# truongp-aws/neuronx-distributed-llama3_2

Hardware: AMD Instinct MI355X
Metric: tokens/sec (whole node) Llama-3-8B TP=8 bf16 training at 1/2/4/8 MI355X (higher is better)
Workload: dtype bf16

## Files before the change

### neuronx_distributed_llama3_2_amd/csrc/dense_gemm.hip

```cpp
#include "common.h"

#include <cstdlib>
#include <type_traits>

namespace nxd {
namespace dg {

constexpr int BM = 256, BN = 256, BK = 64, NT = 512;
constexpr int REG = 16384;
constexpr int BUF = 4 * REG;
constexpr int LDS_BYTES = 2 * BUF;
constexpr int R_ALO = 0, R_AHI = REG, R_BLO = 2 * REG, R_BHI = 3 * REG;

enum Layout { LNT = 0, LTN = 1 };
enum Epi { BF16 = 0, F32_ACC = 1, F32_ATOMIC = 2 };

struct Params {
  const uint16_t* a;
  const uint16_t* b;
  void* c;
  int M, N, K;
  int64_t lda, ldb, ldc;
  int mt, nt;
  int splits;
  int k_per_split;
  int band;
};

typedef __attribute__((address_space(3))) char lds_char_t;
typedef __attribute__((address_space(3))) short4_t lds_short4_t;
__device__ __forceinline__ uint32_t lds_addr(const char* q) { return (uint32_t)(uintptr_t)(const lds_char_t*)q; }

__device__ __forceinline__ void dma16(const void* src, uint32_t lds_dst) {
  uint32_t sv;
  asm volatile("s_mov_b32 %0, m0\n\ts_mov_b32 m0, %2\n\ts_nop 0\n\tglobal_load_lds_dwordx4 %1, off\n\ts_mov_b32 m0, %0"
               : "=&s"(sv) : "v"(src), "s"(lds_dst) : "memory");
}

__device__ __forceinline__ int nt_swz(int r) { return (r >> 1) & 7; }
__device__ __forceinline__ int tn_swz(int t) { return 2 * ((t & 3) | (((t >> 3) & 1) << 2)); }

__device__ __forceinline__ bf16x8_t frag_nt(const char* reg, int r0, int s) {
  const int l = threadIdx.x & 63, r = r0 + (l & 15), ch = (l >> 4) + 4 * s;
  return __builtin_bit_cast(bf16x8_t, *reinterpret_cast<const u32x4_t*>(reg + r * 128 + ((ch ^ nt_swz(r)) << 4)));
}
__device__ __forceinline__ bf16x8_t frag_tn(const char* reg, int f0, int s) {
  const int l = threadIdx.x & 63, g = l >> 4, i = l & 15, q = i >> 2, p = i & 3;
  const int col = f0 + 4 * p, t = 32 * s + 8 * g + q;
  const char* b0 = reg + t * 256 + (((col >> 3) ^ tn_swz(t)) << 4) + 8 * (p & 1);
  const char* b1 = reg + (t + 4) * 256 + (((col >> 3) ^ tn_swz(t + 4)) << 4) + 8 * (p & 1);
  const short4_t lo = __builtin_amdgcn_ds_read_tr16_b64_v4i16((lds_short4_t*)b0);
  const short4_t hi = __builtin_amdgcn_ds_read_tr16_b64_v4i16((lds_short4_t*)b1);
  const short __attribute__((ext_vector_type(8))) a8 = {lo[0], lo[1], lo[2], lo[3], hi[0], hi[1], hi[2], hi[3]};
  return __builtin_bit_cast(bf16x8_t, a8);
}

template <int L>
__device__ __forceinline__ bf16x8_t frag(const char* reg, int x0, int s) {
  if constexpr (L == LNT) return frag_nt(reg, x0, s);
  else return frag_tn(reg, x0, s);
}

__device__ __forceinline__ void barrier() {
  __builtin_amdgcn_sched_barrier(0);
  __builtin_amdgcn_s_barrier();
  __builtin_amdgcn_sched_barrier(0);
}

__device__ __forceinline__ void wait_regions(int younger) {
  switch (younger) {
    case 5: asm volatile("s_waitcnt vmcnt(10)" ::: "memory"); break;
    case 4: asm volatile("s_waitcnt vmcnt(8)" ::: "memory"); break;
    case 3: asm volatile("s_waitcnt vmcnt(6)" ::: "memory"); break;
    case 2: asm volatile("s_waitcnt vmcnt(4)" ::: "memory"); break;
    case 1: asm volatile("s_waitcnt vmcnt(2)" ::: "memory"); break;
    default: asm volatile("s_waitcnt vmcnt(0)" ::: "memory"); break;
  }
}

template <int L, int E, int PIPE>
__global__ void __launch_bounds__(NT, 1) gemm_kernel(Params p) {
  __shared__ __attribute__((aligned(16))) char smem[LDS_BYTES];
  const int tiles = p.mt * p.nt;
  const int id = xcd_remap(blockIdx.x, gridDim.x);
  const int split = id / tiles;
  int rt, ct;
  {
    const int within = id - split * tiles;
    const int kb = p.band, bnd = within / (kb * p.nt), rem = within - bnd * kb * p.nt;
    const int h = min(kb, p.mt - bnd * kb);
    rt = bnd * kb + rem % h;
    ct = rem / h;
  }
  const int m0 = rt * BM, n0 = ct * BN;
  const int k_begin = split * p.k_per_split;
  const int k_end = min(p.K, k_begin + p.k_per_split);
  const int nk = (k_end - k_begin) / BK;

  const int wid = threadIdx.x >> 6, lane = threadIdx.x & 63;
  const int wr = wid >> 2, wc = wid & 3;

  f32x4_t acc[4][4][2];
#pragma unroll
  for (int q = 0; q < 4; ++q)
#pragma unroll
    for (int i = 0; i < 4; ++i)
#pragma unroll
      for (int j = 0; j < 2; ++j) acc[q][i][j] = f32x4_t{0.f, 0.f, 0.f, 0.f};

  const uint16_t* sa[2][2];
// ... 14 lines not shown
      }
    }
  const int64_t adv_a = L == LNT ? (int64_t)BK : (int64_t)BK * p.lda;
  const int64_t adv_b = L == LNT ? (int64_t)BK : (int64_t)BK * p.ldb;
  const uint32_t lds0 = lds_addr(smem);

  auto issue = [&](auto rc, int s) {
    constexpr int R = decltype(rc)::value;
    if (s >= nk) return;
    const uint32_t dst = lds0 + (s & 1) * BUF + (R == 0 ? R_ALO : R == 1 ? R_BLO : R == 2 ? R_BHI : R_AHI) + wid * 2048;
    if constexpr (R == 0 || R == 3) {
      constexpr int h = R == 0 ? 0 : 1;
      const int64_t o = (int64_t)s * adv_a;
      dma16(sa[h][0] + o, __builtin_amdgcn_readfirstlane(dst));
      dma16(sa[h][1] + o, __builtin_amdgcn_readfirstlane(dst + 1024));
    } else {
      constexpr int h = R == 1 ? 0 : 1;
      const int64_t o = (int64_t)s * adv_b;
      dma16(sb[h][0] + o, __builtin_amdgcn_readfirstlane(dst));
      dma16(sb[h][1] + o, __builtin_amdgcn_readfirstlane(dst + 1024));
    }
  };
  const int last = 4 * nk - 1;
  auto wait_for = [&](int need, int max_younger = 4) {
    if (need > last) return;
    wait_regions(min(max_younger, last - need));
  };

  using I0 = std::integral_constant<int, 0>;
  using I1 = std::integral_constant<int, 1>;
  using I2 = std::integral_constant<int, 2>;
  using I3 = std::integral_constant<int, 3>;
  bf16x8_t af[4][2], blo[2][2], bhi[2][2];
  auto mfma_q = [&](auto qc, bf16x8_t (&bf)[2][2]) {
    constexpr int qd = decltype(qc)::value;
    __builtin_amdgcn_s_setprio(1);
#pragma unroll
    for (int s = 0; s < 2; ++s)
#pragma unroll
      for (int i = 0; i < 4; ++i)
#pragma unroll
        for (int j = 0; j < 2; ++j)
          acc[qd][i][j] = __builtin_amdgcn_mfma_f32_16x16x32_bf16(af[i][s], bf[j][s], acc[qd][i][j], 0, 0, 0);
    __builtin_amdgcn_s_setprio(0);
  };

  if constexpr (PIPE == 0) {
  issue(I0{}, 0); issue(I1{}, 0); issue(I2{}, 0); issue(I3{}, 0); issue(I0{}, 1); issue(I1{}, 1);
  wait_for(1);
  barrier();
  const bool grp1 = wr == 1;
  if (grp1) barrier();
  for (int t = 0; t < nk; ++t) {
    const char* buf = smem + (t & 1) * BUF;
    issue(I2{}, t + 1);
#pragma unroll
    for (int i = 0; i < 4; ++i)
#pragma unroll
      for (int s = 0; s < 2; ++s) af[i][s] = frag<L>(buf + R_ALO, wr * 64 + 16 * i, s);
#pragma unroll
    for (int j = 0; j < 2; ++j)
#pragma unroll
      for (int s = 0; s < 2; ++s) blo[j][s] = frag<L>(buf + R_BLO, wc * 32 + 16 * j, s);
    if (grp1) wait_for(4 * t + 2);
    barrier();
    mfma_q(I0{}, blo);
    if (!grp1) wait_for(4 * t + 2);
    barrier();
    issue(I3{}, t + 1);
#pragma unroll
    for (int j = 0; j < 2; ++j)
#pragma unroll
      for (int s = 0; s < 2; ++s) bhi[j][s] = frag<L>(buf + R_BHI, wc * 32 + 16 * j, s);
    if (grp1) wait_for(4 * t + 3);
    barrier();
    mfma_q(I1{}, bhi);
    if (!grp1) wait_for(4 * t + 3);
    barrier();
    issue(I0{}, t + 2);
#pragma unroll
    for (int i = 0; i < 4; ++i)
#pragma unroll
      for (int s = 0; s < 2; ++s) af[i][s] = frag<L>(buf + R_AHI, wr * 64 + 16 * i, s);
    barrier();
    mfma_q(I2{}, bhi);
    barrier();
    issue(I1{}, t + 2);
    if (grp1) wait_for(4 * t + 5);
    barrier();
    mfma_q(I3{}, blo);
    if (!grp1) wait_for(4 * t + 5);
    barrier();
  }
  if (!grp1) barrier();
  } else {
    issue(I0{}, 0); issue(I1{}, 0); issue(I2{}, 0); issue(I3{}, 0); issue(I0{}, 1); issue(I1{}, 1); issue(I2{}, 1);
    wait_for(1, 5);
    barrier();
#pragma unroll
    for (int i = 0; i < 4; ++i)
#pragma unroll
      for (int s = 0; s < 2; ++s) af[i][s] = frag<L>(smem + R_ALO, wr * 64 + 16 * i, s);
#pragma unroll
    for (int j = 0; j < 2; ++j)
#pragma unroll
      for (int s = 0; s < 2; ++s) blo[j][s] = frag<L>(smem + R_BLO, wc * 32 + 16 * j, s);
    wait_for(2);
    barrier();
    for (int t = 0; t < nk; ++t) {
      const char* buf = smem + (t & 1) * BUF;
      const char* nbuf = smem + ((t + 1) & 1) * BUF;
      issue(I3{}, t + 1);
#pragma unroll
      for (int s = 0; s < 2; ++s)
#pragma unroll
        for (int i = 0; i < 4; ++i) {
#pragma unroll
          for (int j = 0; j < 2; ++j)
            acc[0][i][j] = __builtin_amdgcn_mfma_f32_16x16x32_bf16(af[i][s], blo[j][s], acc[0][i][j], 0, 0, 0);
          if (i < 2) bhi[i][s] = frag<L>(buf + R_BHI, wc * 32 + 16 * i, s);
        }
      wait_for(4 * t + 3);
      barrier();
      issue(I0{}, t + 2);
#pragma unroll
      for (int s = 0; s < 2; ++s)
#pragma unroll
        for (int i = 0; i < 4; ++i) {
#pragma unroll
          for (int j = 0; j < 2; ++j)
            acc[1][i][j] = __builtin_amdgcn_mfma_f32_16x16x32_bf16(af[i][s], bhi[j][s], acc[1][i][j], 0, 0, 0);
          af[i][s] = frag<L>(buf + R_AHI, wr * 64 + 16 * i, s);
        }
      barrier();
      issue(I1{}, t + 2);
#pragma unroll
      for (int s = 0; s < 2; ++s)
#pragma unroll
        for (int i = 0; i < 4; ++i)
#pragma unroll
          for (int j = 0; j < 2; ++j)
            acc[2][i][j] = __builtin_amdgcn_mfma_f32_16x16x32_bf16(af[i][s], bhi[j][s], acc[2][i][j], 0, 0, 0);
      wait_for(4 * t + 5);
      barrier();
      issue(I2{}, t + 2);
#pragma unroll
      for (int s = 0; s < 2; ++s)
#pragma unroll
        for (int j = 0; j < 2; ++j) {
#pragma unroll
          for (int i = 0; i < 4; ++i) {
            acc[3][i][j] = __builtin_amdgcn_mfma_f32_16x16x32_bf16(af[i][s], blo[j][s], acc[3][i][j], 0, 0, 0);
            if (j == 1) af[i][s] = frag<L>(nbuf + R_ALO, wr * 64 + 16 * i, s);
          }
          blo[j][s] = frag<L>(nbuf + R_BLO, wc * 32 + 16 * j, s);
        }
      wait_for(4 * t + 6);
      barrier();
    }
  }
  asm volatile("s_waitcnt vmcnt(0)" ::: "memory");
  __syncthreads();

  constexpr int LD = 36;
  float* slab = reinterpret_cast<float*>(smem) + wid * (64 * LD);
  const int crow = 4 * (lane >> 4), ccol = lane & 15;
#pragma unroll
  for (int qd = 0; qd < 4; ++qd) {
    const int rh = (qd == 2 || qd == 3) ? 1 : 0, ch = (qd == 1 || qd == 2) ? 1 : 0;
#pragma unroll
    for (int i = 0; i < 4; ++i)
#pragma unroll
      for (int j = 0; j < 2; ++j)
#pragma unroll
        for (int r = 0; r < 4; ++r) slab[(16 * i + crow + r) * LD + 16 * j + ccol] = acc[qd][i][j][r];
    __builtin_amdgcn_wave_barrier();
    const int row0 = m0 + 128 * rh + 64 * wr, col0 = n0 + 128 * ch + 32 * wc;
    if constexpr (E == F32_ATOMIC) {
      const int col = col0 + (lane & 31);
      float* cp = static_cast<float*>(p.c);
#pragma unroll 8
      for (int rr = 0; rr < 32; ++rr) {
        const int lr = 2 * rr + (lane >> 5), row = row0 + lr;
        const float v = slab[lr * LD + (lane & 31)];
        if (row < p.M && col < p.N) unsafeAtomicAdd(cp + (int64_t)row * p.ldc + col, v);
      }
    } else {
#pragma unroll
      for (int ps = 0; ps < 4; ++ps) {
        const int lr = 16 * ps + (lane >> 2), c8 = 8 * (lane & 3);
        const int row = row0 + lr, col = col0 + c8;
        const f32x4_t v0 = *reinterpret_cast<const f32x4_t*>(slab + lr * LD + c8);
        const f32x4_t v1 = *reinterpret_cast<const f32x4_t*>(slab + lr * LD + c8 + 4);
        if (row < p.M && col < p.N) {
          if constexpr (E == BF16) {
            u32x4_t o;
            o[0] = pack2bf(v0[0], v0[1]); o[1] = pack2bf(v0[2], v0[3]);
            o[2] = pack2bf(v1[0], v1[1]); o[3] = pack2bf(v1[2], v1[3]);
            *reinterpret_cast<u32x4_t*>(static_cast<uint16_t*>(p.c) + (int64_t)row * p.ldc + col) = o;
          } else {
            f32x4_t* cp = reinterpret_cast<f32x4_t*>(static_cast<float*>(p.c) + (int64_t)row * p.ldc + col);
            const f32x4_t c0 = cp[0], c1 = cp[1];
            cp[0] = c0 + v0;
            cp[1] = c1 + v1;
          }
        }
      }
    }
    __builtin_amdgcn_wave_barrier();
  }
}

constexpr int NT4 = 256;

__device__ __forceinline__ int tn4_swz(int t) { return ((t & 3) << 2) | ((t >> 2) & 3); }

template <int L>
__device__ __forceinline__ bf16x8_t frag32(const char* reg, int x0, int ks) {
  const int l = threadIdx.x & 63;
  if constexpr (L == LNT) {
    const int r = x0 + (l & 31), ch = 2 * ks + (l >> 5);
    return __builtin_bit_cast(bf16x8_t, *reinterpret_cast<const u32x4_t*>(reg + r * 128 + ((ch ^ nt_swz(r)) << 4)));
  } else {
    const int g = l >> 4, q = (l >> 2) & 3, pp = l & 3;
    const int t = 16 * ks + 8 * (g >> 1) + q;
    const int ch = (x0 >> 3) + 2 * (g & 1) + (pp >> 1);
    const char* b0 = reg + t * 256 + ((ch ^ tn4_swz(t)) << 4) + 8 * (pp & 1);
    const char* b1 = reg + (t + 4) * 256 + ((ch ^ tn4_swz(t + 4)) << 4) + 8 * (pp & 1);
    const short4_t lo = __builtin_amdgcn_ds_read_tr16_b64_v4i16((lds_short4_t*)b0);
    const short4_t hi = __builtin_amdgcn_ds_read_tr16_b64_v4i16((lds_short4_t*)b1);
    const short __attribute__((ext_vector_type(8))) a8 = {lo[0], lo[1], lo[2], lo[3], hi[0], hi[1], hi[2], hi[3]};
    return __builtin_bit_cast(bf16x8_t, a8);
  }
}

template <int L, int E>
__global__ void __launch_bounds__(NT4, 1) gemm4_kernel(Params p) {
  __shared__ __attribute__((aligned(16))) char smem[LDS_BYTES];
  const int tiles = p.mt * p.nt;
  const int id = xcd_remap(blockIdx.x, gridDim.x);
  const int split = id / tiles;
  int rt, ct;
  {
    const int within = id - split * tiles;
    const int kb = p.band, bnd = within / (kb * p.nt), rem = within - bnd * kb * p.nt;
    const int h = min(kb, p.mt - bnd * kb);
    rt = bnd * kb + rem % h;
    ct = rem / h;
  }
  const int m0 = rt * BM, n0 = ct * BN;
  const int k_begin = split * p.k_per_split;
  const int k_end = min(p.K, k_begin + p.k_per_split);
  const int nk = (k_end - k_begin) / BK;
  const int wid = threadIdx.x >> 6, lane = threadIdx.x & 63;
  const int wr = wid >> 1, wc = wid & 1;

  f32x16_t acc[4][4];
#pragma unroll
  for (int i = 0; i < 4; ++i)
#pragma unroll
    for (int j = 0; j < 4; ++j)
#pragma unroll
      for (int r = 0; r < 16; ++r) acc[i][j][r] = 0.f;

  constexpr int NV = L == LNT ? 2 : 4;
  const uint16_t* sa[NV];
  const uint16_t* sb[NV];
#pragma unroll
  for (int v = 0; v < NV; ++v) {
    if constexpr (L == LNT) {
      const int pr = 8 * (4 * wid + v) + (lane >> 3), c = (lane & 7) ^ nt_swz(pr);
      sa[v] = p.a + (int64_t)(m0 + pr) * p.lda + k_begin + 8 * c;
      sb[v] = p.b + (int64_t)(n0 + pr) * p.ldb + k_begin + 8 * c;
    } else {
      const int pr = 4 * (4 * wid + v) + (lane >> 4), c = (lane & 15) ^ tn4_swz(pr);
      sa[v] = p.a + (int64_t)(k_begin + pr) * p.lda + m0 + 8 * c;
      sb[v] = p.b + (int64_t)(k_begin + pr) * p.ldb + n0 + 8 * c;
    }
  }
  auto pv = [](int j) { return L == LNT ? (j & 1) : j; };
  auto poff = [&](int h, int j, int64_t ld) -> int64_t {
    if constexpr (L == LNT) return (int64_t)(128 * h + 8 * (j & ~1)) * ld;
    else return (int64_t)128 * h;
  };
  const int64_t adv_a = L == LNT ? (int64_t)BK : (int64_t)BK * p.lda;
  const int64_t adv_b = L == LNT ? (int64_t)BK : (int64_t)BK * p.ldb;
  const uint32_t lds0 = lds_addr(smem);
  auto issue_piece = [&](int s, int q) {
    const int r = q >> 2, j = q & 3, h = r & 1;
    const uint32_t dst = lds0 + (s & 1) * BUF + (r == 0 ? R_ALO : r == 1 ? R_AHI : r == 2 ? R_BLO : R_BHI) + wid * 4096 + j * 1024;
    const uint16_t* src = r < 2 ? sa[pv(j)] + (int64_t)s * adv_a + poff(h, j, p.lda)
                                : sb[pv(j)] + (int64_t)s * adv_b + poff(h, j, p.ldb);
    dma16(src, __builtin_amdgcn_readfirstlane(dst));
  };
  const int ra = wr ? R_AHI : R_ALO, rb = wc ? R_BHI : R_BLO;
  bf16x8_t fa0[4], fb0[4], fa1[4], fb1[4];
  auto rd = [&](const char* buf, int ks, bf16x8_t (&fa)[4], bf16x8_t (&fb)[4]) {
#pragma unroll
    for (int i = 0; i < 4; ++i) fa[i] = frag32<L>(buf + ra, 32 * i, ks);
#pragma unroll
    for (int j = 0; j < 4; ++j) fb[j] = frag32<L>(buf + rb, 32 * j, ks);
  };
  auto mm = [&](bf16x8_t (&fa)[4], bf16x8_t (&fb)[4]) {
#pragma unroll
    for (int i = 0; i < 4; ++i)
#pragma unroll
      for (int j = 0; j < 4; ++j) acc[i][j] = __builtin_amdgcn_mfma_f32_32x32x16_bf16(fa[i], fb[j], acc[i][j], 0, 0, 0);
  };

#pragma unroll
  for (int q = 0; q < 16; ++q) issue_piece(0, q);
  if (nk > 1) {
#pragma unroll
    for (int q = 0; q < 16; ++q) issue_piece(1, q);
    asm volatile("s_waitcnt vmcnt(16)" ::: "memory");
  } else {
    asm volatile("s_waitcnt vmcnt(0)" ::: "memory");
  }
  barrier();
  rd(smem, 0, fa0, fb0);
  for (int t = 0; t < nk; ++t) {
    const char* buf = smem + (t & 1) * BUF;
    rd(buf, 1, fa1, fb1);
    mm(fa0, fb0);
    rd(buf, 2, fa0, fb0);
    mm(fa1, fb1);
    rd(buf, 3, fa1, fb1);
    mm(fa0, fb0);
    asm volatile("s_waitcnt lgkmcnt(0)" ::: "memory");
    asm volatile("s_waitcnt vmcnt(0)" ::: "memory");
    barrier();
    rd(smem + ((t + 1) & 1) * BUF, 0, fa0, fb0);
    if (t + 2 < nk) {
#pragma unroll
      for (int q = 0; q < 16; ++q) issue_piece(t + 2, q);
    }
    mm(fa1, fb1);
  }
  asm volatile("s_waitcnt vmcnt(0)" ::: "memory");
  __syncthreads();

  constexpr int LD = 132;
  float* slab = reinterpret_cast<float*>(smem) + wid * (32 * LD);
#pragma unroll
  for (int i = 0; i < 4; ++i) {
#pragma unroll
    for (int j = 0; j < 4; ++j)
#pragma unroll
      for (int r = 0; r < 16; ++r)
        slab[((r & 3) + 8 * (r >> 2) + 4 * (lane >> 5)) * LD + 32 * j + (lane & 31)] = acc[i][j][r];
    __builtin_amdgcn_wave_barrier();
    const int row0 = m0 + 128 * wr + 32 * i, col0 = n0 + 128 * wc;
    if constexpr (E == F32_ATOMIC) {
      float* cp = static_cast<float*>(p.c);
#pragma unroll 2
      for (int rr = 0; rr < 64; ++rr) {
        const int lr = rr >> 1, col = col0 + 64 * (rr & 1) + lane, row = row0 + lr;
        const float v = slab[lr * LD + 64 * (rr & 1) + lane];
        if (row < p.M && col < p.N) unsafeAtomicAdd(cp + (int64_t)row * p.ldc + col, v);
      }
    } else {
#pragma unroll
      for (int ps = 0; ps < 8; ++ps) {
        const int lr = 4 * ps + (lane >> 4), c8 = 8 * (lane & 15);
        const int row = row0 + lr, col = col0 + c8;
        const f32x4_t v0 = *reinterpret_cast<const f32x4_t*>(slab + lr * LD + c8);
        const f32x4_t v1 = *reinterpret_cast<const f32x4_t*>(slab + lr * LD + c8 + 4);
        if (row < p.M && col < p.N) {
          if constexpr (E == BF16) {
            u32x4_t o;
            o[0] = pack2bf(v0[0], v0[1]); o[1] = pack2bf(v0[2], v0[3]);
            o[2] = pack2bf(v1[0], v1[1]); o[3] = pack2bf(v1[2], v1[3]);
            *reinterpret_cast<u32x4_t*>(static_cast<uint16_t*>(p.c) + (int64_t)row * p.ldc + col) = o;
          } else {
            f32x4_t* cp = reinterpret_cast<f32x4_t*>(static_cast<float*>(p.c) + (int64_t)row * p.ldc + col);
            const f32x4_t c0 = cp[0], c1 = cp[1];
            cp[0] = c0 + v0;
            cp[1] = c1 + v1;
          }
        }
      }
    }
    __builtin_amdgcn_wave_barrier();
  }
}

static int g_pipe = -1;

static int env_int(const char* name, int dflt) {
  const char* e = getenv(name);
  return e ? atoi(e) : dflt;
}

}

void dense_gemm_set_pipe(int v) { dg::g_pipe = v; }

// ... 8 lines not shown
    const int64_t cost = (int64_t)ceil_div(tiles * s, 256) * (ceil_div(steps, s) + 6);
    if (cost * 10 < best_cost * 9 && cost < best_cost) {
      best_cost = cost;
      best = s;
    }
  }
  return best;
}

int dense_gemm_launch(int layout, int epi, const void* a, int64_t lda, const void* b, int64_t ldb, void* c, int64_t ldc,
                      int M, int N, int K, int splits, hipStream_t stream) {
  if (M <= 0 || N <= 0 || K <= 0) return 0;
  if (K % dg::BK || N % 8 || lda % 8 || ldb % 8 || ldc % 4) return -1;
  if (layout == dg::LTN && M % 8) return -1;
  if (epi == dg::BF16 && ldc % 8) return -1;
  dg::Params p{};
  p.a = static_cast<const uint16_t*>(a);
  p.b = static_cast<const uint16_t*>(b);
  p.c = c;
  p.M = M; p.N = N; p.K = K;
  p.lda = lda; p.ldb = ldb; p.ldc = ldc;
  p.mt = ceil_div(M, dg::BM);
  p.nt = ceil_div(N, dg::BN);
  const int steps = K / dg::BK;
  if (epi != dg::F32_ATOMIC) splits = 1;
  else if (splits <= 0) splits = dense_gemm_choose_splits(M, N, K);
  splits = splits < 1 ? 1 : (splits > steps ? steps : splits);
  p.k_per_split = ceil_div(steps, splits) * dg::BK;
  p.splits = ceil_div(K, p.k_per_split);
  static const int band = [] { const int v = dg::env_int("NXD_DG_BAND", 8); return v > 0 ? v : 8; }();
  p.band = band;
  const int64_t nwg = (int64_t)p.mt * p.nt * p.splits;
  if (nwg > INT32_MAX) return -2;
  static int pipe_env = dg::env_int("NXD_DG_PIPE", 1);
  int pipe = dg::g_pipe >= 0 ? dg::g_pipe : pipe_env;
  if (pipe == 2 && (M % dg::BM || N % dg::BN)) pipe = 1;
#define NXD_DG_LAUNCH(LY, EP)                                                                                  \
  do {                                                                                                       \
    if (pipe == 2) hipLaunchKernelGGL((dg::gemm4_kernel<LY, EP>), dim3((unsigned)nwg), dim3(dg::NT4), 0, stream, p); \
    else if (pipe) hipLaunchKernelGGL((dg::gemm_kernel<LY, EP, 1>), dim3((unsigned)nwg), dim3(dg::NT), 0, stream, p); \
    else hipLaunchKernelGGL((dg::gemm_kernel<LY, EP, 0>), dim3((unsigned)nwg), dim3(dg::NT), 0, stream, p);      \
  } while (0)
  if (layout == dg::LNT) {
    if (epi == dg::BF16) NXD_DG_LAUNCH(dg::LNT, dg::BF16);
    else if (epi == dg::F32_ACC) NXD_DG_LAUNCH(dg::LNT, dg::F32_ACC);
    else NXD_DG_LAUNCH(dg::LNT, dg::F32_ATOMIC);
  } else {
    if (epi == dg::BF16) NXD_DG_LAUNCH(dg::LTN, dg::BF16);
    else if (epi == dg::F32_ACC) NXD_DG_LAUNCH(dg::LTN, dg::F32_ACC);
    else NXD_DG_LAUNCH(dg::LTN, dg::F32_ATOMIC);
  }
#undef NXD_DG_LAUNCH
  return hipGetLastError() == hipSuccess ? 0 : -3;
}

}
```

### neuronx_distributed_llama3_2_amd/models/llama/modeling_llama.py

```python

from __future__ import annotations

import math
from dataclasses import dataclass
from functools import partial
from typing import Optional

import torch
import torch.nn.functional as F
from torch import nn
from torch.utils.checkpoint import checkpoint

from ... import ops
from ...modules.qkv_linear import GQAQKVColumnParallelLinear
from ...parallel_layers.layer_norm import RMSNorm
from ...parallel_layers.layers import ColumnParallelLinear, ParallelEmbedding, RowParallelLinear
from ...parallel_layers.loss_functions import parallel_cross_entropy
from ...parallel_layers.mappings import gather_from_sequence_parallel_region, scatter_to_sequence_parallel_region
from ...parallel_layers import stream_split
from ...parallel_layers.parallel_state import (get_data_parallel_size, get_pipeline_model_parallel_size,
                                                      get_tensor_model_parallel_size)
from ...parallel_layers.utils import divide


# ... 1 lines not shown

    def __init__(self, loss=None, logits=None):
        super().__init__(loss=loss, logits=logits)

    @property
    def loss(self):
        return self["loss"]

    @property
    def logits(self):
        return self["logits"]


def _init_normal(std, w):
    return nn.init.normal_(w, mean=0.0, std=std)


class LlamaMLP(nn.Module):
    def __init__(self, config, dtype, device):
        super().__init__()
        sp = getattr(config, "sequence_parallel_enabled", False)
        init = partial(_init_normal, config.initializer_range)
        self.gate_up_proj = ColumnParallelLinear(config.hidden_size, 2 * config.intermediate_size, stride=2, bias=False,
                                                 gather_output=False, init_method=init, sequence_parallel_enabled=sp,
                                                 dtype=dtype, device=device)
        self.down_proj = RowParallelLinear(config.intermediate_size, config.hidden_size, bias=False,
                                           input_is_parallel=True, init_method=init, sequence_parallel_enabled=sp,
                                           dtype=dtype, device=device)
        self.selective_checkpoint = getattr(config, "selective_checkpoint_enabled", False)

    def forward(self, x):
        gu = self.gate_up_proj(x)
        if self.selective_checkpoint and self.training:
            h = checkpoint(ops.swiglu, gu, True, use_reentrant=False)
        else:
            h = ops.swiglu(gu, token_major=True)
        return self.down_proj(h)


class LlamaAttention(nn.Module):
    def __init__(self, config, dtype, device, rope_cache):
        super().__init__()
        self.config = config
        self.hidden_size = config.hidden_size
        self.num_heads = config.num_attention_heads
        self.num_kv_heads = getattr(config, "num_key_value_heads", None) or self.num_heads
        self.head_dim = getattr(config, "head_dim", None) or self.hidden_size // self.num_heads
        tp = get_tensor_model_parallel_size()
        kv_mult = getattr(config, "kv_shared_group_size", 1)
        if self.num_kv_heads * kv_mult < tp or (self.num_kv_heads * kv_mult) % tp:
            kv_mult = max(kv_mult, tp // math.gcd(tp, self.num_kv_heads))
        self.kv_mult = kv_mult
        self.num_heads_local = divide(self.num_heads, tp)
        self.num_kv_heads_local = divide(self.num_kv_heads * kv_mult, tp)
        sp = getattr(config, "sequence_parallel_enabled", False)
        init = partial(_init_normal, config.initializer_range)
        self.qkv_proj = GQAQKVColumnParallelLinear(
            self.hidden_size, [self.num_heads * self.head_dim, self.num_kv_heads * self.head_dim],
            bias=getattr(config, "attention_bias", False), gather_output=False, init_method=init,
            sequence_parallel_enabled=sp, kv_size_multiplier=kv_mult, fuse_qkv=True, dtype=dtype, device=device)
        self.o_proj = RowParallelLinear(self.num_heads * self.head_dim, self.hidden_size,
                                        bias=getattr(config, "attention_bias", False), input_is_parallel=True,
                                        init_method=init, sequence_parallel_enabled=sp, dtype=dtype, device=device,
                                        keep_master_weight=kv_mult > 1)
        if kv_mult > 1:
            _regroup_row_parallel(self.o_proj, tp, kv_mult)
        self.rope_cache = rope_cache

    def forward(self, x, key_ranges=None, positions=None):
# ... 44 lines not shown

    def forward(self, hidden_states, residual=None, key_ranges=None, positions=None):
        if residual is None:
            normed = self.input_layernorm(hidden_states)
            residual = hidden_states
        else:
            normed, residual = self.input_layernorm(hidden_states, residual)
        if key_ranges is None and positions is None:
            attn = self.self_attn(normed)
        else:
            attn = self.self_attn(normed, key_ranges, positions)
        normed, residual = self.post_attention_layernorm(attn, residual)
        return self.mlp(normed), residual

    def forward_stages(self, hidden_states, residual=None, key_ranges=None, positions=None):
        if residual is None:
            normed = self.input_layernorm(hidden_states)
            residual = hidden_states
        else:
            normed, residual = self.input_layernorm(hidden_states, residual)
        att = self.self_attn
        qkv = att.qkv_proj.forward_fused(normed)
        yield
        cos_t, sin_t = att.rope_cache.tables(qkv.device)
        o = ops.rope_attention(qkv, cos_t, sin_t, att.num_heads_local, att.num_kv_heads_local, att.head_dim,
                               causal=True, key_ranges=key_ranges, positions=positions)
        attn = att.o_proj(o)
        yield
        normed, residual = self.post_attention_layernorm(attn, residual)
        mlp = self.mlp
        gu = mlp.gate_up_proj(normed)
        yield
        if mlp.selective_checkpoint and self.training:
            h = checkpoint(ops.swiglu, gu, True, use_reentrant=False)
        else:
            h = ops.swiglu(gu, token_major=True)
        out = mlp.down_proj(h)
        yield
        return out, residual


class LlamaModel(nn.Module):
    def __init__(self, config, dtype=torch.bfloat16, device=None):
        super().__init__()
        self.config = config
        sp = getattr(config, "sequence_parallel_enabled", False)
        self.sequence_parallel_enabled = sp and get_tensor_model_parallel_size() > 1
        head_dim = getattr(config, "head_dim", None) or config.hidden_size // config.num_attention_heads
        self.rope_cache = RopeCache(config, head_dim)
        init = partial(_init_normal, config.initializer_range)
        self.embed_tokens = ParallelEmbedding(config.vocab_size, config.hidden_size, init_method=init, dtype=dtype,
                                              device=device, sequence_parallel_enabled=self.sequence_parallel_enabled)
        self.layers = nn.ModuleList([LlamaDecoderLayer(config, dtype, device, self.rope_cache)
                                     for _ in range(config.num_hidden_layers)])
        self.norm = RMSNorm(config.hidden_size, eps=config.rms_norm_eps, sequence_parallel_enabled=sp, dtype=dtype,
                            device=device)
        self.activation_checkpoint = getattr(config, "activation_checkpoint", None)

    def forward(self, input_ids: torch.Tensor, key_ranges=None, positions=None) -> torch.Tensor:
        masked = key_ranges is not None or positions is not None
        ids = input_ids.t().contiguous()
        hidden = self.embed_tokens(ids)
        residual = None
        for layer in self.layers:
            if self.activation_checkpoint == "full" and self.training:
                if masked:
                    res = checkpoint(layer, hidden, residual, key_ranges, positions, use_reentrant=False)
                else:
                    res = checkpoint(layer, hidden, residual, use_reentrant=False)
# ... 153 lines not shown
```

### neuronx_distributed_llama3_2_amd/ops/activations.py

```python

from __future__ import annotations

import os

import torch
import torch.nn.functional as F

from ._ext import ext, use_native


def swiglu_reference(gu: torch.Tensor) -> torch.Tensor:
    g, u = gu.float().chunk(2, dim=-1)
    return (F.silu(g) * u).to(gu.dtype)


_DUAL = os.environ.get("NXD_SWIGLU_DUAL", "1") == "1"
_DUAL_FWD = os.environ.get("NXD_SWIGLU_DUAL_FWD", "1") == "1"


class SwiGLUFunc(torch.autograd.Function):
    @staticmethod
    def forward(ctx, gu, want_t=False, want_grad_t=False):
        gu = gu.contiguous()
        ctx.want_grad_t = want_grad_t
# ... 1 lines not shown
        I = h.shape[-1]
        rows = h.numel() // I if I else 0
        if want_t and rows and rows % 64 == 0 and I % 64 == 0:
            h_t = torch.empty((I, rows), dtype=gu.dtype, device=gu.device)
            ext().swiglu_fwd_dual(gu, h, h_t)
            h._nxd_t, h._nxd_t_ver = h_t, h._version
        else:
            ext().swiglu_fwd(gu, h)
        ctx.save_for_backward(gu)
        return h

    @staticmethod
    def backward(ctx, dh):
        (gu,) = ctx.saved_tensors
        dgu = torch.empty_like(gu)
        I2 = gu.shape[-1]
        rows = gu.numel() // I2 if I2 else 0
        if ctx.want_grad_t and _DUAL and rows and rows % 64 == 0 and (I2 // 2) % 64 == 0:
            dgu_t = torch.empty((I2, rows), dtype=gu.dtype, device=gu.device)
            ext().swiglu_bwd_dual(gu, dh.contiguous(), dgu, dgu_t)
            dgu._nxd_t, dgu._nxd_t_ver = dgu_t, dgu._version
            return dgu, None, None
        ext().swiglu_bwd(gu, dh.contiguous(), dgu)
        return dgu, None, None


def attached_token_major(x: torch.Tensor):
    t = getattr(x, "_nxd_t", None)
    if t is None or getattr(x, "_nxd_t_ver", None) != x._version:
        return None
    return t


def swiglu(gu: torch.Tensor, token_major: bool = False) -> torch.Tensor:
    if use_native(gu):
        train = token_major and torch.is_grad_enabled() and gu.requires_grad
        return SwiGLUFunc.apply(gu, _DUAL_FWD and train, train)
    return swiglu_reference(gu)
```

### neuronx_distributed_llama3_2_amd/ops/gemm.py

```python

from __future__ import annotations

import os

import torch

from ._ext import ext, use_native

_ENABLED = os.environ.get("NXD_TUNED_GEMM", "1") == "1"


def set_overlap_safe(enabled: bool) -> None:
    if not torch.cuda.is_available():
        return
    try:
        ext().gemm_set_no_streamk(1 if enabled else 0)
    except Exception:
        pass


def _native(*t: torch.Tensor) -> bool:
    return _ENABLED and use_native(*t) and all(x.dtype in (torch.bfloat16, torch.float16) for x in t)


# ... 49 lines not shown
_WG_WIDE = 16000


def _use_wgrad_kernel(mg: torch.Tensor, go2: torch.Tensor, x2: torch.Tensor, has_copy: bool = False) -> bool:
    if _WG_KERNEL == "0" or x2 is None or not _native(go2, x2) or mg.dtype != torch.float32:
        return False
    T, M = go2.shape
    N = x2.shape[1]
    if T % 32 or M % 8 or N % 8 or go2.stride(1) != 1 or x2.stride(1) != 1 or mg.stride(1) != 1:
        return False
    if go2.stride(0) % 8 or x2.stride(0) % 8 or go2.data_ptr() % 16 or x2.data_ptr() % 16:
        return False
    return _WG_KERNEL == "1" or M * N / (M + N) < _WG_SKINNY or (not has_copy and max(M, N) >= _WG_WIDE)


_DENSE_WG = os.environ.get("NXD_DENSE_WGRAD", "auto")
_DENSE_WG_SKINNY = 2200.0


def _use_dense_wgrad(mg: torch.Tensor, go2: torch.Tensor, x2, has_copy: bool) -> bool:
    if _DENSE_WG == "0" or x2 is None or not _native(go2, x2) or mg.dtype != torch.float32:
        return False
    T, M = go2.shape
    N = x2.shape[1]
    if T % 64 or M % 8 or N % 8 or go2.stride(1) != 1 or x2.stride(1) != 1 or mg.stride(1) != 1:
        return False
    if go2.stride(0) % 8 or x2.stride(0) % 8 or mg.stride(0) % 4:
        return False
    if go2.data_ptr() % 16 or x2.data_ptr() % 16 or mg.data_ptr() % 16:
        return False
    return _DENSE_WG == "1" or (not has_copy and M * N / (M + N) < _DENSE_WG_SKINNY)


def _dense_wgrad(mg: torch.Tensor, go2: torch.Tensor, x2: torch.Tensor) -> None:
    C = ext()
    T, M = go2.shape
    splits = C.dense_gemm_splits(M, x2.shape[1], T)
    C.dense_gemm(1, 1 if splits == 1 else 2, go2, x2, mg, splits)


def _wgrad_scratch(n: int, dtype, device, tag: str = "") -> torch.Tensor:
    sid = torch.cuda.current_stream(device).stream_id if torch.device(device).type == "cuda" else 0
    key = (dtype, str(device), tag, sid)
    t = _scratch.get(key)
    if t is None or t.numel() < n:
        t = _scratch[key] = torch.empty(n, dtype=dtype, device=device)
    return t[:n]


def wgrad_accumulate_(mg: torch.Tensor, go2: torch.Tensor, x2, go_t: torch.Tensor = None,
                      x_t: torch.Tensor = None) -> None:
    has_copy = go_t is not None or x_t is not None
    if _use_dense_wgrad(mg, go2, x2, has_copy):
        _dense_wgrad(mg, go2, x2)
        return
    if _use_wgrad_kernel(mg, go2, x2, has_copy=has_copy):
        ext().wgrad_gemm(mg, go2, x2, 0)
        return
    if x_t is not None and not (x_t.dim() == 2 and x_t.is_contiguous() and x_t.shape[1] == go2.shape[0]):
        x_t = None
    if x2 is None and not (x_t is not None and _native(go2, x_t) and mg.is_contiguous()
                           and _use_wgrad_t(go2, K=x_t.shape[0])):
        x2 = x_t.t().contiguous()
        x_t = None
    if x2 is None or (_native(go2, x2) and mg.is_contiguous()):
        if x2 is None or _use_wgrad_t(go2, x2):
            T, N = go2.shape[0], go2.shape[1]
            K = x_t.shape[0] if x_t is not None else x2.shape[1]
            if go_t is not None and go_t.shape == (N, T) and go_t.is_contiguous() and go_t.dtype == go2.dtype:
                gt = go_t
            else:
                gt = transpose(go2, out=_wgrad_scratch(N * T, go2.dtype, go2.device, "gt").view(N, T))
            xt = x_t if x_t is not None else transpose(x2, out=_wgrad_scratch(K * T, x2.dtype, x2.device, "xt").view(K, T))
            ext().gemm(gt, xt.t(), mg, None, 1.0, 1.0)
            return
        if _WGRAD_BF16:
            tmp = _wgrad_scratch(mg.numel(), go2.dtype, go2.device).view(mg.shape)
            ext().gemm(go2.t(), x2, tmp, None, 1.0, 0.0)
            mg.add_(tmp)
            return
        ext().gemm(go2.t(), x2, mg, None, 1.0, 1.0)
        return
    if go2.is_cuda:
        torch.addmm(mg, go2.t(), x2, out_dtype=torch.float32, out=mg)
    else:
        mg.add_(go2.t().float().matmul(x2.float()))

# ... 45 lines not shown
```

Baseline: 20860.

## Add scalar-base DMA pipeline variant, drop old pipes, add wide dense wgrad path

Replaces the PIPE==0 and 4-wave gemm4 kernels with a new PIPE=3 pipeline. It uses a scalar base pointer plus precomputed 32-bit per-lane offsets for the global-to-LDS loads, compile-time vmcnt waits and tail specialisation for the last k-tiles, and makes it the default. It falls back to PIPE 1 when leading dimensions are too large for 32-bit offsets. It also adds an optional wide non-split dense wgrad path and lets swiglu skip producing transposed copies when that path would be used. The Python path is gated by an empty floor table, so in auto mode it is effectively off.

```diff
diff --git a/neuronx_distributed_llama3_2_amd/csrc/dense_gemm.hip b/neuronx_distributed_llama3_2_amd/csrc/dense_gemm.hip
--- a/neuronx_distributed_llama3_2_amd/csrc/dense_gemm.hip
+++ b/neuronx_distributed_llama3_2_amd/csrc/dense_gemm.hip
@@ -37,6 +37,11 @@
                : "=&s"(sv) : "v"(src), "s"(lds_dst) : "memory");
 }
 
+__device__ __forceinline__ void dma_region(const char* base, uint32_t off0, uint32_t off1, uint32_t lds_dst) {
+  asm volatile("s_mov_b32 m0, %3\n\ts_nop 0\n\tglobal_load_lds_dwordx4 %1, %0\n\tglobal_load_lds_dwordx4 %2, %0 offset:1024"
+               :: "s"(base), "v"(off0), "v"(off1), "s"(lds_dst) : "memory");
+}
+
 __device__ __forceinline__ int nt_swz(int r) { return (r >> 1) & 7; }
 __device__ __forceinline__ int tn_swz(int t) { return 2 * ((t & 3) | (((t >> 3) & 1) << 2)); }
 
@@ -76,6 +81,11 @@
     case 1: asm volatile("s_waitcnt vmcnt(2)" ::: "memory"); break;
     default: asm volatile("s_waitcnt vmcnt(0)" ::: "memory"); break;
   }
+}
+
+template <int YOUNGER>
+__device__ __forceinline__ void wait_regions_c() {
+  if constexpr (YOUNGER >= 0) asm volatile("s_waitcnt vmcnt(%0)" :: "n"(2 * YOUNGER) : "memory");
 }
 
 template <int L, int E, int PIPE>
@@ -156,68 +166,7 @@
   using I2 = std::integral_constant<int, 2>;
   using I3 = std::integral_constant<int, 3>;
   bf16x8_t af[4][2], blo[2][2], bhi[2][2];
-  auto mfma_q = [&](auto qc, bf16x8_t (&bf)[2][2]) {
-    constexpr int qd = decltype(qc)::value;
-    __builtin_amdgcn_s_setprio(1);
-#pragma unroll
-    for (int s = 0; s < 2; ++s)
-#pragma unroll
-      for (int i = 0; i < 4; ++i)
-#pragma unroll
-        for (int j = 0; j < 2; ++j)
-          acc[qd][i][j] = __builtin_amdgcn_mfma_f32_16x16x32_bf16(af[i][s], bf[j][s], acc[qd][i][j], 0, 0, 0);
-    __builtin_amdgcn_s_setprio(0);
-  };
-
-  if constexpr (PIPE == 0) {
-  issue(I0{}, 0); issue(I1{}, 0); issue(I2{}, 0); issue(I3{}, 0); issue(I0{}, 1); issue(I1{}, 1);
-  wait_for(1);
-  barrier();
-  const bool grp1 = wr == 1;
-  if (grp1) barrier();
-  for (int t = 0; t < nk; ++t) {
-    const char* buf = smem + (t & 1) * BUF;
-    issue(I2{}, t + 1);
-#pragma unroll
-    for (int i = 0; i < 4; ++i)
-#pragma unroll
-      for (int s = 0; s < 2; ++s) af[i][s] = frag<L>(buf + R_ALO, wr * 64 + 16 * i, s);
-#pragma unroll
-    for (int j = 0; j < 2; ++j)
-#pragma unroll
-      for (int s = 0; s < 2; ++s) blo[j][s] = frag<L>(buf + R_BLO, wc * 32 + 16 * j, s);
-    if (grp1) wait_for(4 * t + 2);
-    barrier();
-    mfma_q(I0{}, blo);
-    if (!grp1) wait_for(4 * t + 2);
-    barrier();
-    issue(I3{}, t + 1);
-#pragma unroll
-    for (int j = 0; j < 2; ++j)
-#pragma unroll
-      for (int s = 0; s < 2; ++s) bhi[j][s] = frag<L>(buf + R_BHI, wc * 32 + 16 * j, s);
-    if (grp1) wait_for(4 * t + 3);
-    barrier();
-    mfma_q(I1{}, bhi);
-    if (!grp1) wait_for(4 * t + 3);
-    barrier();
-    issue(I0{}, t + 2);
-#pragma unroll
-    for (int i = 0; i < 4; ++i)
-#pragma unroll
-      for (int s = 0; s < 2; ++s) af[i][s] = frag<L>(buf + R_AHI, wr * 64 + 16 * i, s);
-    barrier();
-    mfma_q(I2{}, bhi);
-    barrier();
-    issue(I1{}, t + 2);
-    if (grp1) wait_for(4 * t + 5);
-    barrier();
-    mfma_q(I3{}, blo);
-    if (!grp1) wait_for(4 * t + 5);
-    barrier();
-  }
-  if (!grp1) barrier();
-  } else {
+  if constexpr (PIPE == 1) {
     issue(I0{}, 0); issue(I1{}, 0); issue(I2{}, 0); issue(I3{}, 0); issue(I0{}, 1); issue(I1{}, 1); issue(I2{}, 1);
     wait_for(1, 5);
     barrier();
@@ -282,6 +231,131 @@
       wait_for(4 * t + 6);
       barrier();
     }
+  } else {
+    const int widu = __builtin_amdgcn_readfirstlane(wid);
+    uint32_t oa[2][2], ob[2][2];
+#pragma unroll
+    for (int h = 0; h < 2; ++h)
+#pragma unroll
+      for (int j = 0; j < 2; ++j) {
+        const int piece = 2 * widu + j, bias = j == 0 ? 1024 : 0;
+        if constexpr (L == LNT) {
+          const int pr = 8 * piece + (lane >> 3), c = (lane & 7) ^ nt_swz(pr);
+          oa[h][j] = (uint32_t)(((int64_t)(min(m0 + 128 * h + pr, p.M - 1) - m0) * p.lda + 8 * c) * 2 + bias);
+          ob[h][j] = (uint32_t)(((int64_t)(min(n0 + 128 * h + pr, p.N - 1) - n0) * p.ldb + 8 * c) * 2 + bias);
+        } else {
+          const int pr = 4 * piece + (lane >> 4), c = (lane & 15) ^ tn_swz(pr);
+          oa[h][j] = (uint32_t)(((int64_t)pr * p.lda + min(m0 + 128 * h + 8 * c, p.M - 8) - m0) * 2 + bias);
+          ob[h][j] = (uint32_t)(((int64_t)pr * p.ldb + min(n0 + 128 * h + 8 * c, p.N - 8) - n0) * 2 + bias);
+        }
+      }
+    const char* pa;
+    const char* pb;
+    if constexpr (L == LNT) {
+      pa = reinterpret_cast<const char*>(p.a + (int64_t)m0 * p.lda + k_begin) - 1024;
+      pb = reinterpret_cast<const char*>(p.b + (int64_t)n0 * p.ldb + k_begin) - 1024;
+    } else {
+      pa = reinterpret_cast<const char*>(p.a + (int64_t)k_begin * p.lda + m0) - 1024;
+      pb = reinterpret_cast<const char*>(p.b + (int64_t)k_begin * p.ldb + n0) - 1024;
+    }
+    const int64_t ba = 2 * adv_a, bb = 2 * adv_b;
+    const uint32_t ldsw = lds0 + widu * 2048;
+    auto issue3 = [&](auto rc, const char* ta, const char* tb, int par) {
+      constexpr int R = decltype(rc)::value;
+      const uint32_t dst = ldsw + par * BUF + (R == 0 ? R_ALO : R == 1 ? R_BLO : R == 2 ? R_BHI : R_AHI);
+      if constexpr (R == 0) dma_region(ta, oa[0][0], oa[0][1], dst);
+      else if constexpr (R == 3) dma_region(ta, oa[1][0], oa[1][1], dst);
+      else if constexpr (R == 1) dma_region(tb, ob[0][0], ob[0][1], dst);
+      else dma_region(tb, ob[1][0], ob[1][1], dst);
+    };
+    auto ktile = [&](auto remc, int t, const char* ta, const char* tb) {
+      constexpr int REM = decltype(remc)::value;
+      const int par = t & 1;
+      const char* buf = smem + par * BUF;
+      const char* nbuf = smem + (par ^ 1) * BUF;
+      if constexpr (REM >= 2) issue3(I3{}, ta + ba, tb + bb, par ^ 1);
+#pragma unroll
+      for (int s = 0; s < 2; ++s)
+#pragma unroll
+        for (int i = 0; i < 4; ++i) {
+#pragma unroll
+          for (int j = 0; j < 2; ++j)
+            acc[0][i][j] = __builtin_amdgcn_mfma_f32_16x16x32_bf16(af[i][s], blo[j][s], acc[0][i][j], 0, 0, 0);
+          if (i < 2) bhi[i][s] = frag<L>(buf + R_BHI, wc * 32 + 16 * i, s);
+          __builtin_amdgcn_sched_barrier(0);
+        }
+      wait_regions_c<(4 * REM - 4 < 4 ? 4 * REM - 4 : 4)>();
+      barrier();
+      if constexpr (REM >= 3) issue3(I0{}, ta + 2 * ba, tb + 2 * bb, par);
+#pragma unroll
+      for (int s = 0; s < 2; ++s)
+#pragma unroll
+        for (int i = 0; i < 4; ++i) {
+#pragma unroll
+          for (int j = 0; j < 2; ++j)
+            acc[1][i][j] = __builtin_amdgcn_mfma_f32_16x16x32_bf16(af[i][s], bhi[j][s], acc[1][i][j], 0, 0, 0);
+          af[i][s] = frag<L>(buf + R_AHI, wr * 64 + 16 * i, s);
+          __builtin_amdgcn_sched_barrier(0);
+        }
+      barrier();
+      if constexpr (REM >= 3) issue3(I1{}, ta + 2 * ba, tb + 2 * bb, par);
+#pragma unroll
+      for (int s = 0; s < 2; ++s)
+#pragma unroll
+        for (int i = 0; i < 4; ++i)
+#pragma unroll
+          for (int j = 0; j < 2; ++j)
+            acc[2][i][j] = __builtin_amdgcn_mfma_f32_16x16x32_bf16(af[i][s], bhi[j][s], acc[2][i][j], 0, 0, 0);
+      wait_regions_c<(4 * REM - 6 < 4 ? 4 * REM - 6 : 4)>();
+      barrier();
+      if constexpr (REM >= 3) issue3(I2{}, ta + 2 * ba, tb + 2 * bb, par);
+#pragma unroll
+      for (int s = 0; s < 2; ++s)
+#pragma unroll
+        for (int j = 0; j < 2; ++j) {
+#pragma unroll
+          for (int i = 0; i < 4; ++i) {
+            acc[3][i][j] = __builtin_amdgcn_mfma_f32_16x16x32_bf16(af[i][s], blo[j][s], acc[3][i][j], 0, 0, 0);
+            if constexpr (REM >= 2) {
+              if (j == 1) af[i][s] = frag<L>(nbuf + R_ALO, wr * 64 + 16 * i, s);
+              __builtin_amdgcn_sched_barrier(0);
+            }
+          }
+          if constexpr (REM >= 2) {
+            blo[j][s] = frag<L>(nbuf + R_BLO, wc * 32 + 16 * j, s);
+            __builtin_amdgcn_sched_barrier(0);
+          }
+        }
+      wait_regions_c<(4 * REM - 7 < 4 ? 4 * REM - 7 : 4)>();
+      barrier();
+    };
+    issue3(I0{}, pa, pb, 0); issue3(I1{}, pa, pb, 0); issue3(I2{}, pa, pb, 0); issue3(I3{}, pa, pb, 0);
+    if (nk > 1) { issue3(I0{}, pa + ba, pb + bb, 1); issue3(I1{}, pa + ba, pb + bb, 1); issue3(I2{}, pa + ba, pb + bb, 1); }
+    wait_for(1, 5);
+    barrier();
+#pragma unroll
+    for (int i = 0; i < 4; ++i)
+#pragma unroll
+      for (int s = 0; s < 2; ++s) af[i][s] = frag<L>(smem + R_ALO, wr * 64 + 16 * i, s);
+#pragma unroll
+    for (int j = 0; j < 2; ++j)
+#pragma unroll
+      for (int s = 0; s < 2; ++s) blo[j][s] = frag<L>(smem + R_BLO, wc * 32 + 16 * j, s);
+    wait_for(2);
+    barrier();
+    int t = 0;
+    for (; t < nk - 2; ++t) {
+      ktile(I3{}, t, pa, pb);
+      pa += ba;
+      pb += bb;
+    }
+    if (nk >= 2) {
+      ktile(I2{}, t, pa, pb);
+      pa += ba;
+      pb += bb;
+      ++t;
+    }
+    ktile(I1{}, t, pa, pb);
   }
   asm volatile("s_waitcnt vmcnt(0)" ::: "memory");
   __syncthreads();
@@ -313,180 +387,6 @@
 #pragma unroll
       for (int ps = 0; ps < 4; ++ps) {
         const int lr = 16 * ps + (lane >> 2), c8 = 8 * (lane & 3);
-        const int row = row0 + lr, col = col0 + c8;
-        const f32x4_t v0 = *reinterpret_cast<const f32x4_t*>(slab + lr * LD + c8);
-        const f32x4_t v1 = *reinterpret_cast<const f32x4_t*>(slab + lr * LD + c8 + 4);
-        if (row < p.M && col < p.N) {
-          if constexpr (E == BF16) {
-            u32x4_t o;
-            o[0] = pack2bf(v0[0], v0[1]); o[1] = pack2bf(v0[2], v0[3]);
-            o[2] = pack2bf(v1[0], v1[1]); o[3] = pack2bf(v1[2], v1[3]);
-            *reinterpret_cast<u32x4_t*>(static_cast<uint16_t*>(p.c) + (int64_t)row * p.ldc + col) = o;
-          } else {
-            f32x4_t* cp = reinterpret_cast<f32x4_t*>(static_cast<float*>(p.c) + (int64_t)row * p.ldc + col);
-            const f32x4_t c0 = cp[0], c1 = cp[1];
-            cp[0] = c0 + v0;
-            cp[1] = c1 + v1;
-          }
-        }
-      }
-    }
-    __builtin_amdgcn_wave_barrier();
-  }
-}
-
-constexpr int NT4 = 256;
-
-__device__ __forceinline__ int tn4_swz(int t) { return ((t & 3) << 2) | ((t >> 2) & 3); }
-
-template <int L>
-__device__ __forceinline__ bf16x8_t frag32(const char* reg, int x0, int ks) {
-  const int l = threadIdx.x & 63;
-  if constexpr (L == LNT) {
-    const int r = x0 + (l & 31), ch = 2 * ks + (l >> 5);
-    return __builtin_bit_cast(bf16x8_t, *reinterpret_cast<const u32x4_t*>(reg + r * 128 + ((ch ^ nt_swz(r)) << 4)));
-  } else {
-    const int g = l >> 4, q = (l >> 2) & 3, pp = l & 3;
-    const int t = 16 * ks + 8 * (g >> 1) + q;
-    const int ch = (x0 >> 3) + 2 * (g & 1) + (pp >> 1);
-    const char* b0 = reg + t * 256 + ((ch ^ tn4_swz(t)) << 4) + 8 * (pp & 1);
-    const char* b1 = reg + (t + 4) * 256 + ((ch ^ tn4_swz(t + 4)) << 4) + 8 * (pp & 1);
-    const short4_t lo = __builtin_amdgcn_ds_read_tr16_b64_v4i16((lds_short4_t*)b0);
-    const short4_t hi = __builtin_amdgcn_ds_read_tr16_b64_v4i16((lds_short4_t*)b1);
-    const short __attribute__((ext_vector_type(8))) a8 = {lo[0], lo[1], lo[2], lo[3], hi[0], hi[1], hi[2], hi[3]};
-    return __builtin_bit_cast(bf16x8_t, a8);
-  }
-}
-
-template <int L, int E>
-__global__ void __launch_bounds__(NT4, 1) gemm4_kernel(Params p) {
-  __shared__ __attribute__((aligned(16))) char smem[LDS_BYTES];
-  const int tiles = p.mt * p.nt;
-  const int id = xcd_remap(blockIdx.x, gridDim.x);
-  const int split = id / tiles;
-  int rt, ct;
-  {
-    const int within = id - split * tiles;
-    const int kb = p.band, bnd = within / (kb * p.nt), rem = within - bnd * kb * p.nt;
-    const int h = min(kb, p.mt - bnd * kb);
-    rt = bnd * kb + rem % h;
-    ct = rem / h;
-  }
-  const int m0 = rt * BM, n0 = ct * BN;
-  const int k_begin = split * p.k_per_split;
-  const int k_end = min(p.K, k_begin + p.k_per_split);
-  const int nk = (k_end - k_begin) / BK;
-  const int wid = threadIdx.x >> 6, lane = threadIdx.x & 63;
-  const int wr = wid >> 1, wc = wid & 1;
-
-  f32x16_t acc[4][4];
-#pragma unroll
-  for (int i = 0; i < 4; ++i)
-#pragma unroll
-    for (int j = 0; j < 4; ++j)
-#pragma unroll
-      for (int r = 0; r < 16; ++r) acc[i][j][r] = 0.f;
-
-  constexpr int NV = L == LNT ? 2 : 4;
-  const uint16_t* sa[NV];
-  const uint16_t* sb[NV];
-#pragma unroll
-  for (int v = 0; v < NV; ++v) {
-    if constexpr (L == LNT) {
-      const int pr = 8 * (4 * wid + v) + (lane >> 3), c = (lane & 7) ^ nt_swz(pr);
-      sa[v] = p.a + (int64_t)(m0 + pr) * p.lda + k_begin + 8 * c;
-      sb[v] = p.b + (int64_t)(n0 + pr) * p.ldb + k_begin + 8 * c;
-    } else {
-      const int pr = 4 * (4 * wid + v) + (lane >> 4), c = (lane & 15) ^ tn4_swz(pr);
-      sa[v] = p.a + (int64_t)(k_begin + pr) * p.lda + m0 + 8 * c;
-      sb[v] = p.b + (int64_t)(k_begin + pr) * p.ldb + n0 + 8 * c;
-    }
-  }
-  auto pv = [](int j) { return L == LNT ? (j & 1) : j; };
-  auto poff = [&](int h, int j, int64_t ld) -> int64_t {
-    if constexpr (L == LNT) return (int64_t)(128 * h + 8 * (j & ~1)) * ld;
-    else return (int64_t)128 * h;
-  };
-  const int64_t adv_a = L == LNT ? (int64_t)BK : (int64_t)BK * p.lda;
-  const int64_t adv_b = L == LNT ? (int64_t)BK : (int64_t)BK * p.ldb;
-  const uint32_t lds0 = lds_addr(smem);
-  auto issue_piece = [&](int s, int q) {
-    const int r = q >> 2, j = q & 3, h = r & 1;
-    const uint32_t dst = lds0 + (s & 1) * BUF + (r == 0 ? R_ALO : r == 1 ? R_AHI : r == 2 ? R_BLO : R_BHI) + wid * 4096 + j * 1024;
-    const uint16_t* src = r < 2 ? sa[pv(j)] + (int64_t)s * adv_a + poff(h, j, p.lda)
-                                : sb[pv(j)] + (int64_t)s * adv_b + poff(h, j, p.ldb);
-    dma16(src, __builtin_amdgcn_readfirstlane(dst));
-  };
-  const int ra = wr ? R_AHI : R_ALO, rb = wc ? R_BHI : R_BLO;
-  bf16x8_t fa0[4], fb0[4], fa1[4], fb1[4];
-  auto rd = [&](const char* buf, int ks, bf16x8_t (&fa)[4], bf16x8_t (&fb)[4]) {
-#pragma unroll
-    for (int i = 0; i < 4; ++i) fa[i] = frag32<L>(buf + ra, 32 * i, ks);
-#pragma unroll
-    for (int j = 0; j < 4; ++j) fb[j] = frag32<L>(buf + rb, 32 * j, ks);
-  };
-  auto mm = [&](bf16x8_t (&fa)[4], bf16x8_t (&fb)[4]) {
-#pragma unroll
-    for (int i = 0; i < 4; ++i)
-#pragma unroll
-      for (int j = 0; j < 4; ++j) acc[i][j] = __builtin_amdgcn_mfma_f32_32x32x16_bf16(fa[i], fb[j], acc[i][j], 0, 0, 0);
-  };
-
-#pragma unroll
-  for (int q = 0; q < 16; ++q) issue_piece(0, q);
-  if (nk > 1) {
-#pragma unroll
-    for (int q = 0; q < 16; ++q) issue_piece(1, q);
-    asm volatile("s_waitcnt vmcnt(16)" ::: "memory");
-  } else {
-    asm volatile("s_waitcnt vmcnt(0)" ::: "memory");
-  }
-  barrier();
-  rd(smem, 0, fa0, fb0);
-  for (int t = 0; t < nk; ++t) {
-    const char* buf = smem + (t & 1) * BUF;
-    rd(buf, 1, fa1, fb1);
-    mm(fa0, fb0);
-    rd(buf, 2, fa0, fb0);
-    mm(fa1, fb1);
-    rd(buf, 3, fa1, fb1);
-    mm(fa0, fb0);
-    asm volatile("s_waitcnt lgkmcnt(0)" ::: "memory");
-    asm volatile("s_waitcnt vmcnt(0)" ::: "memory");
-    barrier();
-    rd(smem + ((t + 1) & 1) * BUF, 0, fa0, fb0);
-    if (t + 2 < nk) {
-#pragma unroll
-      for (int q = 0; q < 16; ++q) issue_piece(t + 2, q);
-    }
-    mm(fa1, fb1);
-  }
-  asm volatile("s_waitcnt vmcnt(0)" ::: "memory");
-  __syncthreads();
-
-  constexpr int LD = 132;
-  float* slab = reinterpret_cast<float*>(smem) + wid * (32 * LD);
-#pragma unroll
-  for (int i = 0; i < 4; ++i) {
-#pragma unroll
-    for (int j = 0; j < 4; ++j)
-#pragma unroll
-      for (int r = 0; r < 16; ++r)
-        slab[((r & 3) + 8 * (r >> 2) + 4 * (lane >> 5)) * LD + 32 * j + (lane & 31)] = acc[i][j][r];
-    __builtin_amdgcn_wave_barrier();
-    const int row0 = m0 + 128 * wr + 32 * i, col0 = n0 + 128 * wc;
-    if constexpr (E == F32_ATOMIC) {
-      float* cp = static_cast<float*>(p.c);
-#pragma unroll 2
-      for (int rr = 0; rr < 64; ++rr) {
-        const int lr = rr >> 1, col = col0 + 64 * (rr & 1) + lane, row = row0 + lr;
-        const float v = slab[lr * LD + 64 * (rr & 1) + lane];
-        if (row < p.M && col < p.N) unsafeAtomicAdd(cp + (int64_t)row * p.ldc + col, v);
-      }
-    } else {
-#pragma unroll
-      for (int ps = 0; ps < 8; ++ps) {
-        const int lr = 4 * ps + (lane >> 4), c8 = 8 * (lane & 15);
         const int row = row0 + lr, col = col0 + c8;
         const f32x4_t v0 = *reinterpret_cast<const f32x4_t*>(slab + lr * LD + c8);
         const f32x4_t v1 = *reinterpret_cast<const f32x4_t*>(slab + lr * LD + c8 + 4);
@@ -561,14 +461,13 @@
   p.band = band;
   const int64_t nwg = (int64_t)p.mt * p.nt * p.splits;
   if (nwg > INT32_MAX) return -2;
-  static int pipe_env = dg::env_int("NXD_DG_PIPE", 1);
+  static int pipe_env = dg::env_int("NXD_DG_PIPE", 3);
   int pipe = dg::g_pipe >= 0 ? dg::g_pipe : pipe_env;
-  if (pipe == 2 && (M % dg::BM || N % dg::BN)) pipe = 1;
+  if (pipe != 1 && (lda >= (1 << 22) || ldb >= (1 << 22))) pipe = 1;
 #define NXD_DG_LAUNCH(LY, EP)                                                                                  \
   do {                                                                                                       \
-    if (pipe == 2) hipLaunchKernelGGL((dg::gemm4_kernel<LY, EP>), dim3((unsigned)nwg), dim3(dg::NT4), 0, stream, p); \
-    else if (pipe) hipLaunchKernelGGL((dg::gemm_kernel<LY, EP, 1>), dim3((unsigned)nwg), dim3(dg::NT), 0, stream, p); \
-    else hipLaunchKernelGGL((dg::gemm_kernel<LY, EP, 0>), dim3((unsigned)nwg), dim3(dg::NT), 0, stream, p);      \
+    if (pipe == 1) hipLaunchKernelGGL((dg::gemm_kernel<LY, EP, 1>), dim3((unsigned)nwg), dim3(dg::NT), 0, stream, p); \
+    else hipLaunchKernelGGL((dg::gemm_kernel<LY, EP, 3>), dim3((unsigned)nwg), dim3(dg::NT), 0, stream, p);      \
   } while (0)
   if (layout == dg::LNT) {
     if (epi == dg::BF16) NXD_DG_LAUNCH(dg::LNT, dg::BF16);
diff --git a/neuronx_distributed_llama3_2_amd/models/llama/modeling_llama.py b/neuronx_distributed_llama3_2_amd/models/llama/modeling_llama.py
--- a/neuronx_distributed_llama3_2_amd/models/llama/modeling_llama.py
+++ b/neuronx_distributed_llama3_2_amd/models/llama/modeling_llama.py
@@ -57,9 +57,9 @@
     def forward(self, x):
         gu = self.gate_up_proj(x)
         if self.selective_checkpoint and self.training:
-            h = checkpoint(ops.swiglu, gu, True, use_reentrant=False)
-        else:
-            h = ops.swiglu(gu, token_major=True)
+            h = checkpoint(ops.swiglu, gu, True, self.gate_up_proj.weight.shape[1], use_reentrant=False)
+        else:
+            h = ops.swiglu(gu, token_major=True, hidden=self.gate_up_proj.weight.shape[1])
         return self.down_proj(h)
 
 
@@ -170,9 +170,9 @@
         gu = mlp.gate_up_proj(normed)
         yield
         if mlp.selective_checkpoint and self.training:
-            h = checkpoint(ops.swiglu, gu, True, use_reentrant=False)
-        else:
-            h = ops.swiglu(gu, token_major=True)
+            h = checkpoint(ops.swiglu, gu, True, mlp.gate_up_proj.weight.shape[1], use_reentrant=False)
+        else:
+            h = ops.swiglu(gu, token_major=True, hidden=mlp.gate_up_proj.weight.shape[1])
         out = mlp.down_proj(h)
         yield
         return out, residual
diff --git a/neuronx_distributed_llama3_2_amd/ops/activations.py b/neuronx_distributed_llama3_2_amd/ops/activations.py
--- a/neuronx_distributed_llama3_2_amd/ops/activations.py
+++ b/neuronx_distributed_llama3_2_amd/ops/activations.py
@@ -57,8 +57,16 @@
     return t
 
 
-def swiglu(gu: torch.Tensor, token_major: bool = False) -> torch.Tensor:
+def swiglu(gu: torch.Tensor, token_major: bool = False, hidden: int = None) -> torch.Tensor:
     if use_native(gu):
         train = token_major and torch.is_grad_enabled() and gu.requires_grad
-        return SwiGLUFunc.apply(gu, _DUAL_FWD and train, train)
+        want_t, want_grad_t = _DUAL_FWD and train, train
+        if train and hidden:
+            from .gemm import dense_wgrad_wide
+
+            I2 = gu.shape[-1]
+            rows = gu.numel() // I2 if I2 else 0
+            want_t = want_t and not dense_wgrad_wide(rows, hidden, I2 // 2)
+            want_grad_t = want_grad_t and not dense_wgrad_wide(rows, I2, hidden)
+        return SwiGLUFunc.apply(gu, want_t, want_grad_t)
     return swiglu_reference(gu)
diff --git a/neuronx_distributed_llama3_2_amd/ops/gemm.py b/neuronx_distributed_llama3_2_amd/ops/gemm.py
--- a/neuronx_distributed_llama3_2_amd/ops/gemm.py
+++ b/neuronx_distributed_llama3_2_amd/ops/gemm.py
@@ -105,10 +105,35 @@
     return _DENSE_WG == "1" or (not has_copy and M * N / (M + N) < _DENSE_WG_SKINNY)
 
 
-def _dense_wgrad(mg: torch.Tensor, go2: torch.Tensor, x2: torch.Tensor) -> None:
+_DENSE_WG_WIDE = os.environ.get("NXD_DENSE_WGRAD_WIDE", "auto")
+_DENSE_WG_WIDE_FLOOR = {}
+
+
+def dense_wgrad_wide(T: int, M: int, N: int) -> bool:
+    if _DENSE_WG_WIDE == "0" or not _ENABLED or T <= 0 or T % 64 or M % 8 or N % 8:
+        return False
+    if _DENSE_WG_WIDE == "1":
+        return True
+    floor = _DENSE_WG_WIDE_FLOOR.get((M, N))
+    return floor is not None and T >= floor
+
+
+def _use_dense_wgrad_wide(mg: torch.Tensor, go2: torch.Tensor, x2) -> bool:
+    if x2 is None or not _native(go2, x2) or mg.dtype != torch.float32 or go2.dim() != 2 or x2.dim() != 2:
+        return False
+    if go2.stride(1) != 1 or x2.stride(1) != 1 or mg.stride(1) != 1:
+        return False
+    if go2.stride(0) % 8 or x2.stride(0) % 8 or mg.stride(0) % 4:
+        return False
+    if go2.data_ptr() % 16 or x2.data_ptr() % 16 or mg.data_ptr() % 16:
+        return False
+    return dense_wgrad_wide(go2.shape[0], go2.shape[1], x2.shape[1])
+
+
+def _dense_wgrad(mg: torch.Tensor, go2: torch.Tensor, x2: torch.Tensor, split_k: bool = True) -> None:
     C = ext()
     T, M = go2.shape
-    splits = C.dense_gemm_splits(M, x2.shape[1], T)
+    splits = C.dense_gemm_splits(M, x2.shape[1], T) if split_k else 1
     C.dense_gemm(1, 1 if splits == 1 else 2, go2, x2, mg, splits)
 
 
@@ -126,6 +151,9 @@
     has_copy = go_t is not None or x_t is not None
     if _use_dense_wgrad(mg, go2, x2, has_copy):
         _dense_wgrad(mg, go2, x2)
+        return
+    if _use_dense_wgrad_wide(mg, go2, x2):
+        _dense_wgrad(mg, go2, x2, split_k=False)
         return
     if _use_wgrad_kernel(mg, go2, x2, has_copy=has_copy):
         ext().wgrad_gemm(mg, go2, x2, 0)
```

Result: no change. 20900 (median of 3 runs) (+0.2%).
